# hsp-iit/roft

Measured on AMD Instinct MI355X. Metric: tracker frames/sec per object (640x480) + ADD-S vs CPU ref, higher is better.
Workload: dtype f64; 1 GPU; BASELINE config #4: 640x480, CV_32FC2 flow grid 1, 64 objects in total, 64 per GPU (sharded by object, no data-path collective; result rows all-gathered over RCCL at N > 1), masks+poses at 5 fps with 6-frame delay, flow-aided masks, re-sync and outlier rejection on, frames submitted in batches of at most 8; objects_per_gpu=64, objects_total=64, width=640, height=480, batch_frames=8, ranks=1, backend=nccl

## Files before the change

### roft_amd/csrc/batch_plan.h

```cpp
#pragma once

#include <cstdlib>

namespace roft {
namespace host {

constexpr int kPlanLanes = 2;

struct SchedKnobs {
    int handoff_mode = 1;
    int prep_mode = 1;
    int part_mode = 1;
    int feat_mask_mode = 1;
    int lanes_wait_skf = 1;
    int early_lanes = 1;
    int ctrl_ingest = 1;
    int gather_copy = 1;
    int outlier_steady_div = 2;
    bool host_prof = false;
    bool host_prof_per_batch = false;
    bool one_stream = false;
};

inline SchedKnobs knobs_from_env()
{
    SchedKnobs k;
    auto num = [](const char* name, int& v) { const char* s = getenv(name); if (s) v = atoi(s); return s != nullptr; };
    num("ROFT_HANDOFF", k.handoff_mode);
    num("ROFT_PREP_AHEAD", k.prep_mode);
    num("ROFT_MASK_PART_GATE", k.part_mode);
    num("ROFT_FEAT_ON_MASK", k.feat_mask_mode);
    if (!num("ROFT_LANES_WAIT_SKF", k.lanes_wait_skf) && getenv("ROCPROF_COUNTER_COLLECTION")) k.handoff_mode = 0;
    num("ROFT_EARLY_LANES", k.early_lanes);
    num("ROFT_CTRL_INGEST", k.ctrl_ingest);
    num("ROFT_GATHER_COPY", k.gather_copy);
    num("ROFT_OUTLIER_STEADY_DIV", k.outlier_steady_div);
    const char* hp = getenv("ROFT_HOST_PROF");
    k.host_prof = hp && hp[0] == '1';
    k.host_prof_per_batch = k.host_prof && hp[1] == '+';
    const char* one = getenv("ROFT_ONE_STREAM");
    k.one_stream = one && one[0] == '1';
    return k;
}

struct SubmitFacts {
    int T = 1;
    bool had_uploads = false;
    bool produced_flows = false;
    unsigned plain_mask_frames = 0;
    int label_sets = 0;
    int pose_masks = 0;
    int pose_resolve = 0;
    bool any_feat = false, any_feat_now = false;
    bool feat_dep_in_batch = false;
    int n_segments[kPlanLanes] = {1, 1};
    bool lin_any[kPlanLanes] = {false, false};
    int lane_objs[kPlanLanes] = {0, 0}, lane_old_first[kPlanLanes] = {0, 0};
    int relabel_wait[kPlanLanes] = {-1, -1};
};

struct PlanInputs : SubmitFacts {
    SchedKnobs knobs;
    bool multi = true;
    bool timing = false;
    int timing_level = 2;
    bool wait_value_ok = true;
    bool have_skf_started = true;
    int n_obj = 0, cus = 256;
    int batch_counter = 0, idle_mark = 0, lead = 6, completed_batches = 0;
    int outlier_bands_per_alternative = 0;
    bool conflict_free = false;
    bool up_stream_distinct = true;
    bool feat_used_two_back = false;
    bool vel_used_prev = false;
    bool done_used_relabel[kPlanLanes] = {false, false};
    int quality_frames = 0;
};

enum class Signal {
    none,
    stop,
    record,
};
// ... 17 lines not shown
    Signal ev_done = Signal::none;
};

struct BatchPlan {
    bool steady = false, handoff = false;
    bool early_lanes = false;
    bool prep = false;
    bool prep_waits_mask = false, prep_waits_feat = false;
    bool wait_up = false;
    bool try_fused = false;
    bool label_ingest = false;
    bool pose_silhouettes = false;
    bool pose_resolve = false;
    Signal ev_ctrl = Signal::none, ev_prep = Signal::none;
    bool part_gate = false;
    Signal ev_mask = Signal::none;
    FeatRun feat = FeatRun::none;
    Signal ev_feat = Signal::none;
    VelWait vel_waits = VelWait::none;
    bool feat_waits_mask = false;
    Signal ev_skf = Signal::none, ev_vel = Signal::none;
    LanePlan lane[kPlanLanes];
    int outlier_div = 1;
    bool quality = false;
    bool quality_waits_mask = false;
    bool quality_waits_lane = false;
    Signal ev_quality = Signal::none;
};

template <class AloneFn>
// ... 23 lines not shown
    }

    p.prep = batch && in.up_stream_distinct && by_mode(k.prep_mode, p.steady, !cus_to_spare);
    p.prep_waits_mask = p.prep && in.batch_counter >= 2;
    p.prep_waits_feat = p.prep_waits_mask && in.feat_used_two_back;
    p.wait_up = multi && (in.had_uploads || in.produced_flows) && !p.prep;
    p.try_fused = k.ctrl_ingest != 0 && !p.prep && in.plain_mask_frames != 0 && !in.timing;
    p.ev_ctrl = (multi && (in.T == 1 || any_early)) ? Signal::stop : Signal::none;
    p.label_ingest = in.label_sets > 0;
    p.pose_silhouettes = in.pose_masks > 0;
    p.pose_resolve = p.pose_silhouettes && in.pose_resolve > 0;
    p.ev_prep = !p.prep ? Signal::none
                : (full || (in.plain_mask_frames == 0 && !p.label_ingest && !p.pose_silhouettes)) ? Signal::record : Signal::stop;

    p.part_gate = batch && by_mode(k.part_mode, !p.steady, cus_to_spare);
    p.ev_mask = ends(multi);

    const bool feat_behind_skf = batch && !(k.feat_mask_mode == 2 || (k.feat_mask_mode == 1 && 16 * in.n_obj <= in.cus));
    p.feat = !in.any_feat ? FeatRun::none : feat_behind_skf ? FeatRun::behind_skf : FeatRun::mask_stream;
    p.ev_feat = ends(multi && p.feat == FeatRun::mask_stream);

    p.vel_waits = !multi ? VelWait::none : in.T == 1 ? VelWait::ev_ctrl : p.part_gate ? VelWait::ev_part : VelWait::ev_mask;
    p.feat_waits_mask = p.feat == FeatRun::behind_skf && p.part_gate;
    const bool lanes_wait_skf = p.feat == FeatRun::behind_skf && k.lanes_wait_skf != 0 && !own_sets;
    p.ev_skf = ends(lanes_wait_skf);
    p.ev_vel = ends(multi);

    const bool lanes_wait_feat = p.ev_feat != Signal::none && (in.T > 1 || in.any_feat_now);
    for (int l = 0; l < kPlanLanes; ++l) {
        LanePlan& lp = p.lane[l];
// ... 22 lines not shown

    p.outlier_div = (in.outlier_bands_per_alternative == 0 && p.steady && k.outlier_steady_div > 1) ? k.outlier_steady_div : 1;
    return p;
}

enum class PrepLaunch { none, mask_ingest, label_ingest, pose_silhouettes, pose_resolve };
inline PrepLaunch prep_last_launch(const BatchPlan& p, unsigned plain_mask_frames)
{
    return p.pose_resolve ? PrepLaunch::pose_resolve
           : p.pose_silhouettes ? PrepLaunch::pose_silhouettes
           : p.label_ingest ? PrepLaunch::label_ingest
           : plain_mask_frames ? PrepLaunch::mask_ingest : PrepLaunch::none;
}
inline int pose_silhouette_launches(const BatchPlan& p) { return p.pose_resolve ? 2 : p.pose_silhouettes ? 1 : 0; }

}
}
```

### roft_amd/csrc/engine_step.hip

```cpp
#include "engine_internal.h"

__global__ void ctrl_upload_kernel(const uint4* __restrict__ src, EngineArrays a, size_t n16, int reset)
{
    uint4* dst = reinterpret_cast<uint4*>(a.ctrl);
    const size_t i0 = (size_t)blockIdx.x * blockDim.x + threadIdx.x, stride = (size_t)gridDim.x * blockDim.x;
    for (size_t i = i0; i < n16; i += stride) dst[i] = src[i];
    if (reset)
        for (size_t i = i0; i < (size_t)a.T * a.n_obj; i += stride) roft::mask_reset_tables(a, i);
}


static hipEvent_t push_mark(roft_engine* e, const char* name, int which)
{
    const size_t idx = e->tmark.size();
    while (e->tev.size() <= idx) {
        hipEvent_t ev;
        (void)hipEventCreate(&ev);
        e->tev.push_back(ev);
    }
    int id = -1;
    if (name) {
        for (size_t i = 0; i < e->tnames_s.size(); ++i)
            if (e->tnames_s[i] == name) id = (int)i;
        if (id < 0) { e->tnames_s.push_back(name); id = (int)e->tnames_s.size() - 1; }
// ... 57 lines not shown
    roft_engine* e = q.e;
    const PendingBatch& pb = e->pending;
    const BatchPlan& p = q.p;
    const EngineArrays& a = q.a;
    hipStream_t s = e->stream, sp = p.prep ? e->up_stream : s;
    if (p.wait_up) TRY(q.wait(s, q.cur.ev_up));
    if (p.prep_waits_mask) {
        BatchSlot& two_back = e->slot_of(e->batch_counter - 2);
        TRY(q.wait(sp, two_back.ev_mask));
        if (p.prep_waits_feat) TRY(q.wait(sp, two_back.ev_feat));
    }
    tmark(e, nullptr, p.prep ? 4 : 0);
    static_assert(sizeof(FrameCtrl) % 16 == 0, "FrameCtrl is copied in 16-byte units");
    const size_t n16 = (sizeof(FrameCtrl) * (size_t)a.n_obj * a.T + (p.label_ingest ? pb.label_table_bytes : 0)) / 16;
    const hipEvent_t ctrl_stop = Enqueue::stop(p.ev_ctrl, q.cur.ev_ctrl);
    const PrepLaunch last_launch = prep_last_launch(p, pb.facts.plain_mask_frames);
    auto label_ingest = [&]() -> int {
        LabelIngestArgs la;
        la.sets = reinterpret_cast<const LabelSet*>(a.ctrl + (size_t)a.n_obj * a.T);
        la.members = reinterpret_cast<const LabelMember*>(la.sets + pb.label_sets.size());
        la.planes = a.planes;
        la.plane_words = a.plane_words;
        la.obj_stride = (size_t)kPlaneSlotsTotal * 2 * a.plane_words;
        la.slot0 = a.slot_new;
        la.mrec = a.mrec;
        la.n_obj = a.n_obj;
        la.n_grp = a.cam.W * a.cam.H / 64;
        launch_label_ingest(la, (int)pb.label_sets.size(), sp, last_launch == PrepLaunch::label_ingest ? Enqueue::stop(p.ev_prep, q.cur.ev_prep) : nullptr);
        ++q.launches;
        CHECK_LAUNCH("label image ingest");
// ... 30 lines not shown
            sa.zpairs = pm.zpairs.p + (size_t)(e->batch_counter & 1) * kMaxBatch * e->cfg.max_objects;
        }
        const int slot = e->batch_counter % roft_engine::kBatchRing;
        const hipEvent_t plan_stop = Enqueue::stop(p.ev_prep, q.cur.ev_prep);
        if (!p.prep) tmark(e, nullptr, 0);
        const int launched = launch_pose_silhouette(sa, n_frames, a.max_verts, 0, 1, sp, pm.ev_start[slot], plan_stop ? plan_stop : pm.ev_stop[slot]);
        if (launched != pose_silhouette_launches(p))
            return fail(ROFT_ERR_INVALID, "pose masks: the image does not fit the kernel's bit window");
        pm.last_slot = slot;
        pm.last_timed = plan_stop == nullptr;
        q.launches += launched;
        CHECK_LAUNCH(p.pose_resolve ? "pose silhouettes: clear, draw and resolve" : "pose silhouettes");
        if (!p.prep) tmark(e, "pose_silhouettes", 0);
        return ROFT_OK;
    };
    if (p.try_fused && launch_ctrl_ingest(q.cur.stage, a, n16, pb.facts.plain_mask_frames, sp, ctrl_stop)) {
        ++q.launches;
        CHECK_LAUNCH("FrameCtrl upload + mask ingest");
        if (p.label_ingest) TRY(label_ingest());
        return p.pose_silhouettes ? pose_silhouettes() : ROFT_OK;
    }
    hipExtLaunchKernelGGL(ctrl_upload_kernel, dim3((unsigned)std::min<size_t>((n16 + 255) / 256, 64)), dim3(256), 0, sp, nullptr, ctrl_stop, 0,
                          reinterpret_cast<const uint4*>(q.cur.stage), a, n16, 1);
    ++q.launches;
    CHECK_LAUNCH("FrameCtrl upload");
    int last = -1;
    for (int t = 0; t < a.T; ++t)
        if (pb.facts.plain_mask_frames & (1u << t)) last = t;
    for (int t = 0; t <= last; ++t)
        if (pb.facts.plain_mask_frames & (1u << t)) {
            launch_mask_ingest(a, t, sp, (t == last && last_launch == PrepLaunch::mask_ingest) ? Enqueue::stop(p.ev_prep, q.cur.ev_prep) : nullptr);
            ++q.launches;
        }
    CHECK_LAUNCH("mask ingest");
    if (p.label_ingest) TRY(label_ingest());
    if (p.pose_silhouettes) TRY(pose_silhouettes());
    if (p.prep) {
        TRY(q.signalled(p.ev_prep, q.cur.ev_prep, sp));
        tmark(e, "mask_prepare", 4);
        TRY(q.wait(s, q.cur.ev_prep));
    }
    return ROFT_OK;
}

static int enqueue_mask_frames(Enqueue& q)
{
    roft_engine* e = q.e;
    const BatchPlan& p = q.p;
    hipStream_t s = e->stream;
    tmark(e, nullptr, 0);
    q.launches += launch_mask_chain(q.a, e->cfg.mask_frames_between, e->cfg.flow_aided_segmentation, e->pending.new_mask_frames, s,
                                    Enqueue::stop(p.ev_mask, q.cur.ev_mask), p.part_gate ? q.cur.ev_part : nullptr);
    CHECK_LAUNCH("mask chain");
    tmark(e, "mask_chain", 0);
    TRY(q.signalled(p.ev_mask, q.cur.ev_mask, s));
    q.cur.feat_used = p.ev_feat != Signal::none;
    if (p.feat == FeatRun::mask_stream) {
        launch_features(q.a, s, Enqueue::stop(p.ev_feat, q.cur.ev_feat), e->pending.feat_frames);
        ++q.launches;
        CHECK_LAUNCH("features");
        tmark(e, "features", 0);
        TRY(q.signalled(p.ev_feat, q.cur.ev_feat, s));
    }
    return ROFT_OK;
}

static int enqueue_velocity(Enqueue& q)
{
// ... 100 lines not shown
    eq.last_slot = slot;
    return q.signalled(p.ev_quality, eq.ev_done[slot], sp);
}

static PlanInputs plan_inputs(roft_engine* e)
{
    PlanInputs in;
    static_cast<SubmitFacts&>(in) = e->pending.facts;
    in.knobs = e->knobs;
    in.multi = e->multi();
    in.timing = e->timing;
    in.timing_level = e->timing_level;
    in.wait_value_ok = e->wait_value_ok;
    in.have_skf_started = e->arr.skf_started.p != nullptr;
    in.n_obj = e->arr.a.n_obj;
    in.cus = device_cu_count();
    in.batch_counter = e->batch_counter; in.idle_mark = e->idle_mark; in.lead = e->lead; in.completed_batches = e->completed_batches;
    in.outlier_bands_per_alternative = e->cfg.outlier_bands_per_alternative;
    in.conflict_free = e->streams && e->streams->conflicts == 0;
    in.up_stream_distinct = e->up_stream != e->stream;
    if (e->quality.enabled) (void)quality_frames_of_batch(e, &in.quality_frames);
    in.feat_used_two_back = e->batch_counter >= 2 && e->slot_of(e->batch_counter - 2).feat_used;
    in.vel_used_prev = e->batch_counter >= 1 && e->slot_of(e->batch_counter - 1).vel_used;
    for (int l = 0; l < kNumLin; ++l) in.done_used_relabel[l] = in.relabel_wait[l] >= 0 && e->slot_of(in.relabel_wait[l]).done_used[1 - l];
    return in;
}

int step_batch(roft_engine* e)
{
    const PendingBatch& pb = e->pending;
// ... 112 lines not shown
```

### roft_amd/csrc/engine_submit.hip

```cpp
#include "engine_internal.h"

static void take_feat_slot(Sched& o, FrameCtrl& c)
{
    if (c.feat_write < 0) { c.feat_write = o.feat_next; o.feat_next = (o.feat_next + 1) % kFeatRing; }
    o.feat_slot = c.feat_write;
}

bool build_pose_program(const roft_config& cfg, Sched& o, const roft_frame_input& in, FrameCtrl& c)
{
    const int slot = o.frame_idx % kTwistRing;
    c.twist_slot = slot;
    int n = 0;
    bool overflow = false;
    auto add = [&](StepDesc sd) { if (n < kMaxSteps) c.steps[n++] = sd; else overflow = true; };
    auto vel_pop_front = [&]() { std::memmove(o.vel_buf, o.vel_buf + 1, sizeof(int) * (size_t)(--o.n_vel)); };

    const bool has_vel = cfg.use_velocity != 0;
    const bool is_pose = cfg.use_pose && in.pose_valid;
    int type = ROFT_MEAS_NONE;
    if (has_vel && is_pose) type = ROFT_MEAS_POSE_VELOCITY;
    else if (has_vel) type = ROFT_MEAS_VELOCITY;
    else if (is_pose) type = ROFT_MEAS_POSE;
    if (has_vel) {
        if (o.n_vel == kTwistRing) vel_pop_front();
// ... 429 lines not shown

static int schedule_mask_source(roft_engine* e, const FrameJob& j, const ImageSizes& sz, const DevInputs& d)
{
    PendingBatch& pb = e->pending;
    HostObject& ho = j.ho;
    Sched& o = ho.s;
    FrameCtrl& c = j.c;
    c.slot_prev = (o.frame_idx + kPlaneSlots - 1) % kPlaneSlots;
    c.slot_cur = o.frame_idx % kPlaneSlots;
    const EnginePoseMasks& pm = e->pose_masks;
    const bool enrolled = pm.enabled && (ho.pose_masks || (pm.all && has_mesh(e->h_params[j.id])));
    const bool from_pose = enrolled && !d.mask && !d.labels && (j.in.pose_valid || o.track_frames == 0);
    const bool has_mask = d.mask || d.labels || from_pose;
    c.has_new_mask = has_mask ? 1 : 0;
    c.new_mask = static_cast<const uint8_t*>(d.mask);
    if (has_mask) pb.new_mask_frames |= 1u << j.t;
    if (d.mask) pb.facts.plain_mask_frames |= 1u << j.t;
    if (d.labels) {
        c.label = j.lm->label;
        c.label_type = j.lm->label_type;
        int si = -1;
        for (size_t i = pb.label_sets.size(); i-- > 0 && pb.label_sets[i].t == j.t;)
            if (pb.label_sets[i].img == d.labels && pb.label_sets[i].type == j.lm->label_type) { si = (int)i; break; }
        if (si < 0) {
            LabelSet ls{};
            ls.img = d.labels; ls.type = j.lm->label_type; ls.t = j.t;
            pb.label_sets.push_back(ls);
            pb.label_members.emplace_back();
            si = pb.facts.label_sets++;
        }
        pb.label_members[si].push_back(LabelMember{j.id, j.lm->label});
    }
    if (from_pose) {
        c.label_type = kMaskFromPose;
        pb.pose_mask_frames |= 1u << j.t;
        pb.facts.pose_masks++;
    }
    if (has_mask && !o.seg_available) { o.seg_available = true; c.first_mask = 1; }
    if (!o.seg_available)
        return fail(ROFT_ERR_STATE, "no segmentation mask delivered yet: the first frame must carry one (or the object be enrolled with roft_engine_enable_pose_masks)");
    const bool valid_flow = d.flow && !o.of_first_frame;
    o.of_first_frame = false;
    if (valid_flow) {
        const int keep = std::min(o.n_hist, e->hist_cap - 1);
        std::memmove(o.hist + 1, o.hist, sizeof(FlowEntry) * (size_t)keep);
        o.hist[0] = FlowEntry{d.flow, o.frame_idx, -1, o.depth_prev};
        o.n_hist = keep + 1;
        o.flows_since_mask++;
        o.flows_buffered = std::min(o.flows_buffered + 1, kMaxFlowHist);
    }
    for (int k0 = 0; k0 < o.n_hist; ++k0) {
        FlowEntry& fe = o.hist[k0];
        if (fe.owned >= 0 || o.frame_idx - fe.frame < e->hist_cap) continue;
// ... 534 lines not shown
```

### roft_amd/csrc/k_mask.hip

```cpp
#include <algorithm>
#include <initializer_list>

#include "roft_device.h"

namespace roft {

__device__ __forceinline__ void bytes_to_bits(uint32_t w, int shift, unsigned long long& nz, unsigned long long& ob)
{
#pragma unroll
    for (int k = 0; k < 4; ++k) {
        const uint32_t v = (w >> (8 * k)) & 0xFFu;
        nz |= (unsigned long long)(v != 0u) << (shift + k);
        ob |= (unsigned long long)(v > 1u) << (shift + k);
    }
}

__device__ __forceinline__ void ingest_group(const uint4* src, int g, uint2* nz, uint2* ob, int& count, int& ones)
{
    unsigned long long bnz = 0, bob = 0;
    uint4 v[4];
#pragma unroll
    for (int q = 0; q < 4; ++q) v[q] = src[(size_t)g * 4 + q];
#pragma unroll
    for (int q = 0; q < 4; ++q) {
// ... 23 lines not shown
        atomicAdd(&r.new_count, count);
        if (ones) atomicAdd(&r.new_ones, ones);
    }
}

__global__ __launch_bounds__(256) void mask_ingest_kernel(EngineArrays a, int t)
{
    ROFT_RESIDENT(a, RK_MASK_INGEST);
    const int obj = blockIdx.y;
    const FrameCtrl& c = frame_ctrl(a, t, obj);
    if (!c.has_new_mask || c.label_type) return;
    ingest_delivered(a, c, t, obj, blockIdx.x);
}

__global__ __launch_bounds__(256) void ctrl_ingest_kernel(const uint4* __restrict__ src, EngineArrays a, size_t n16, int copy_blocks,
                                                          int chunks, unsigned frames_packed)
{
    if ((int)blockIdx.x < copy_blocks) {
        uint4* dst = reinterpret_cast<uint4*>(a.ctrl);
        const size_t stride = (size_t)copy_blocks * blockDim.x;
        for (size_t i = (size_t)blockIdx.x * blockDim.x + threadIdx.x; i < n16; i += stride) dst[i] = src[i];
        return;
    }
    ROFT_RESIDENT(a, RK_MASK_INGEST);
    const int w = (int)blockIdx.x - copy_blocks;
    const int chunk = w % chunks, rest = w / chunks, obj = rest % a.n_obj, fi = rest / a.n_obj;
    const int t = (int)((frames_packed >> (4 * fi)) & 15u);
    const FrameCtrl& c = reinterpret_cast<const FrameCtrl*>(src)[(size_t)t * a.n_obj + obj];
    if (!c.has_new_mask || c.label_type) return;
    ingest_delivered(a, c, t, obj, chunk);
}

bool launch_ctrl_ingest(const void* staging, const EngineArrays& a, size_t n16, unsigned new_mask_frames, hipStream_t s, hipEvent_t stop)
{
    unsigned packed = 0;
    int n_frames = 0;
    for (int t = 0; t < a.T && t < 16; ++t)
        if (new_mask_frames & (1u << t)) {
            if (n_frames >= 8) return false;
            packed |= (unsigned)t << (4 * n_frames++);
        }
    const int n_grp = a.cam.W * a.cam.H / 64, chunks = (n_grp + 255) / 256;
    const int copy_blocks = (int)std::min<size_t>((n16 + 255) / 256, 64);
    const unsigned grid = (unsigned)copy_blocks + (unsigned)n_frames * (unsigned)a.n_obj * (unsigned)chunks;
    hipExtLaunchKernelGGL(ctrl_ingest_kernel, dim3(grid), dim3(256), 0, s, nullptr, stop, 0, reinterpret_cast<const uint4*>(staging), a, n16,
                          copy_blocks, chunks, packed);
    return true;
}

void launch_mask_ingest(const EngineArrays& a, int t, hipStream_t s, hipEvent_t stop)
{
    const int n_grp = a.cam.W * a.cam.H / 64;
    hipExtLaunchKernelGGL(mask_ingest_kernel, dim3((n_grp + 255) / 256, a.n_obj), dim3(256), 0, s, nullptr, stop, 0, a, t);
}

__device__ __forceinline__ uint32_t eq_bits_u8(uint32_t w, uint32_t rep)
{
    const uint32_t x = w ^ rep;
    const uint32_t z = ~(((x & 0x7F7F7F7Fu) + 0x7F7F7F7Fu) | x | 0x7F7F7F7Fu);
    return ((z >> 7) * 0x01020408u) >> 24;
}
// ... 68 lines not shown
__global__ void mask_reset_kernel(EngineArrays a)
{
    mask_reset_tables(a, (size_t)blockIdx.x * blockDim.x + threadIdx.x);
}

void launch_mask_reset(const EngineArrays& a, hipStream_t s)
{
    hipLaunchKernelGGL(mask_reset_kernel, dim3(((a.T + 1) * a.n_obj + 255) / 256), dim3(256), 0, s, a);
}

constexpr int kFrameThreads = 256, kFreshThreads = 128;

struct MaskShared {
    int bbox[4];
    int n_list;
    unsigned long long w00[2];
    const void* flows[kMaxFlowHist];
};

struct ChaseGeo {
    int W, H, cols, grid;
    float grid_f, scale;
    float inv_grid, inv_scale;
    int mode;
};

__host__ __device__ inline ChaseGeo make_chase_geo(const DevCamera& cam, const DevFlowFmt& f)
{
    ChaseGeo g;
    g.W = cam.W; g.H = cam.H; g.cols = f.cols; g.grid = f.grid;
// ... 339 lines not shown
    if (flow_aided) {
        r.mode = decide_mode(c, new_slot, prev.fbuf_n, new_count, frames_between, r.src_slot, r.n_flows);
        r.fbuf_n = next_fbuf(c, prev.fbuf_n, new_count, r.mode, frames_between);
    } else {
        r.mode = 0;
        r.src_slot = c.has_new_mask ? new_slot : c.slot_prev;
        r.n_flows = 0;
        r.fbuf_n = 0;
    }
    r.src_binary = (r.src_slot >= kSlotNew) ? new_binary : prev.binary;
    r.binary = r.src_binary;
    return r;
}

#ifdef ROFT_MASK_PROFILE
#define MTICK(i) do { __syncthreads(); if (threadIdx.x == 0) atomicMax((unsigned long long*)&a.state[blockIdx.y].dbg[(i)], (unsigned long long)wall_clock64()); } while (0)
#else
#define MTICK(i) do {} while (0)
#endif

template <int FT, int THREADS>
__global__ __launch_bounds__(THREADS) __attribute__((amdgpu_waves_per_eu(4, 8)))
void mask_frame_kernel(EngineArrays a, int t, int frames_between, int flow_aided, int grp_per_wg, int margin, int win_cap)
{
#ifdef ROFT_MASK_PROFILE
    if (threadIdx.x == 0) atomicMax((unsigned long long*)&a.state[blockIdx.y].dbg[8], (unsigned long long)((1ll << 62) - wall_clock64()));
#endif
    ROFT_RESIDENT(a, THREADS == kFreshThreads ? RK_MASK_FRESH_EMPTY : RK_MASK_FRAME_EMPTY);
    extern __shared__ __attribute__((aligned(16))) unsigned char smem[];
    __shared__ MaskShared S;
    __shared__ FrameCtrl s_c;
    __shared__ MaskRec s_rec[2];
    static_assert(sizeof(MaskRec) == 32, "two 16-byte loads per record");
    uint32_t* s_win = reinterpret_cast<uint32_t*>(smem);
    uint32_t* s_list = s_win + win_cap;
    uint2* s_words = reinterpret_cast<uint2*>(s_list + THREADS);
    const int obj = blockIdx.y, q = blockIdx.x;
    const int W = a.cam.W, H = a.cam.H, wpr = a.cam.wpr, n_grp = (W * H) >> 6;
    const int tid = threadIdx.x;
    const int g0 = q * grp_per_wg, g1 = min(n_grp, g0 + grp_per_wg);
    const int r_lo = max(0, (g0 * 64) / W - margin), r_hi = min(H - 1, (g1 * 64 - 1) / W + margin);
    const int win_off = r_lo * wpr, win_words = min(win_cap, (r_hi - r_lo + 1) * wpr);
    stage_ctrl(&s_c, frame_ctrl(a, t, obj));
    if (tid >= THREADS / 2 && tid < THREADS / 2 + 4) {
        const int k = tid - THREADS / 2;
        const MaskRec* prev = (t == 0) ? a.mrec_carry + obj : a.mrec + (size_t)t * a.n_obj + obj;
        reinterpret_cast<uint4*>(s_rec)[k] = (k >= 2) ? reinterpret_cast<const uint4*>(a.mrec + (size_t)(t + 1) * a.n_obj + obj)[k & 1]
                                                      : reinterpret_cast<const uint4*>(prev)[k & 1];
    }
    const int guess_prev = a.slot_prev0 >= 0 ? (a.slot_prev0 + t) % kPlaneSlots : -1, guess_new = a.slot_new + t;
    const ROFT_GLOBAL unsigned long long* pl_prev = guess_prev >= 0 ? (const ROFT_GLOBAL unsigned long long*)(a.planes + plane_offset(a, obj, guess_prev, 1)) : nullptr;
    const ROFT_GLOBAL unsigned long long* pl_new = (const ROFT_GLOBAL unsigned long long*)(a.planes + plane_offset(a, obj, guess_new, 1));
    unsigned long long w_prev = 0ull, w_new = 0ull;
    if (g0 + tid < g1) {
        if (pl_prev) w_prev = pl_prev[g0 + tid];
        w_new = pl_new[g0 + tid];
    }
    if (tid == THREADS * 3 / 4) { S.w00[0] = pl_prev ? pl_prev[0] : 0ull; S.w00[1] = pl_new[0]; }
    for (int i = tid; i < win_words; i += THREADS) s_win[i] = 0u;
    if (tid == 0) S.n_list = 0;
    __syncthreads();
    MTICK(4);
    const FrameCtrl& c = s_c;
    const MaskRec r = decide_frame(s_rec[0], s_rec[1], a.slot_new + t, c, frames_between, flow_aided);
    if (q == 0 && tid == 0) a.mrec[(size_t)(t + 1) * a.n_obj + obj] = r;
    if (tid < kMaxFlowHist) S.flows[tid] = (tid < r.n_flows) ? c.flow[tid] : nullptr;
    MTICK(0);
    const size_t sh0 = (size_t)2 * g0, sh_n = (size_t)2 * (g1 - g0);
    plane_fill(a.planes + plane_offset(a, obj, (c.slot_cur + 1) % kPlaneSlots, 1) + sh0, 0u, sh_n);
    MTICK(5);
    const uint32_t* src = a.planes + plane_offset(a, obj, r.src_slot, 1);
    uint32_t* dst = a.planes + plane_offset(a, obj, c.slot_cur, 1);
    if (!r.src_binary) {
        if (q == 0 && tid == 0) atomicOr(&a.mask_general[obj], 1u << t);
        return;
    }
    if (r.mode == 0) {
        plane_copy(dst + sh0, src + sh0, sh_n);
        return;
    }
    const bool from_guess = r.src_slot == guess_prev || r.src_slot == guess_new;
    const unsigned long long w00 = from_guess ? S.w00[r.src_slot == guess_new ? 1 : 0] : *reinterpret_cast<const unsigned long long*>(src);
    if (r.mode == 2 && (w00 & 1ull)) {
        plane_fill(dst + sh0, ~0u, sh_n);
        return;
    }
    MTICK(6);
    const ChaseGeo geo = make_chase_geo(a.cam, a.ffmt);
// ... 24 lines not shown
        }
        __syncthreads();
        MTICK(1);
        if (S.n_list > 0) ROFT_RESIDENT_AS(a, THREADS == kFreshThreads ? RK_MASK_FRESH : RK_MASK_FRAME);
        propagate_binary<FT, THREADS / 64>(geo, plane2, s_list, S.n_list, r.n_flows, r.mode == 1, S.flows, tgt, s_words);
    }
    __syncthreads();
    MTICK(2);
    for (int i = tid; i < win_words; i += THREADS) {
        const uint32_t v = s_win[i];
        if (v) atomicOr(&dst[win_off + i], v);
    }
    MTICK(3);
}

constexpr int kMaskThreads = 256;
constexpr int kMaskWaves = kMaskThreads / 64;
constexpr int kGeneralList = 16384;
template <int FT>
__global__ __launch_bounds__(kMaskThreads) void mask_general_kernel(EngineArrays a, int final_launch)
{
    extern __shared__ __attribute__((aligned(16))) unsigned char smem[];
    __shared__ MaskShared S;
    uint32_t* s_list = reinterpret_cast<uint32_t*>(smem);
    const int obj = blockIdx.x;
    const int W = a.cam.W, H = a.cam.H, npix = W * H, n_grp = npix >> 6;
    const int tid = threadIdx.x, lane = tid & 63;
    ROFT_RESIDENT(a, RK_MASK_GENERAL);
    if (final_launch && tid < a.T) {
        MaskRec& r0 = a.mrec[(size_t)(tid + 1) * a.n_obj + obj];
        r0.new_count = 0;
        r0.new_ones = 0;
    }
    const unsigned todo = a.mask_general[obj];
    if (!todo) return;
    __syncthreads();
    if (tid == 0) a.mask_general[obj] = 0u;
    for (int t = 0; t < a.T; ++t) {
        if (!((todo >> t) & 1u)) continue;
        const MaskRec r = a.mrec[(size_t)(t + 1) * a.n_obj + obj];
        const FrameCtrl& c = frame_ctrl(a, t, obj);
        const uint32_t* snz = a.planes + plane_offset(a, obj, r.src_slot, 0);
        const uint32_t* sob = a.planes + plane_offset(a, obj, r.src_slot, 1);
        uint32_t* dnz = a.planes + plane_offset(a, obj, c.slot_cur, 0);
        uint32_t* dob = a.planes + plane_offset(a, obj, c.slot_cur, 1);
        if (r.mode == 0) {
            plane_copy(dnz, snz, a.plane_words);
            plane_copy(dob, sob, a.plane_words);
        } else {
            const bool bg_nz = (r.mode == 2) && (snz[0] & 1u), bg_ob = (r.mode == 2) && (sob[0] & 1u);
            if (tid < kMaxFlowHist) S.flows[tid] = (tid < r.n_flows) ? c.flow[tid] : nullptr;
            if (tid == 0) { S.n_list = 0; S.bbox[0] = INT32_MAX; S.bbox[1] = INT32_MAX; S.bbox[2] = -1; S.bbox[3] = -1; }
            __syncthreads();
            const uint2* plane2 = reinterpret_cast<const uint2*>(snz);
            int32_t* map = a.map + (size_t)obj * npix;
            for (int c0 = 0; c0 < n_grp; c0 += kGeneralList) {
                const int c1 = min(n_grp, c0 + kGeneralList);
                for (int g0 = c0; g0 < c1; g0 += kMaskThreads) {
// ... 22 lines not shown
                        obb = (sob[m >> 5] >> (m & 31)) & 1u;
                    }
                }
                const unsigned long long b1 = __ballot(nzb), b2 = __ballot(obb);
                if (lane == 0) {
                    reinterpret_cast<uint2*>(dnz)[g] = make_uint2((uint32_t)b1, (uint32_t)(b1 >> 32));
                    reinterpret_cast<uint2*>(dob)[g] = make_uint2((uint32_t)b2, (uint32_t)(b2 >> 32));
                }
            }
        }
        __syncthreads();
    }
}

int launch_mask_chain(const EngineArrays& a, int frames_between, int flow_aided, unsigned new_mask_frames, hipStream_t s, hipEvent_t stop,
                      hipEvent_t stop_early)
{
    const int n_grp = a.cam.W * a.cam.H / 64;
    constexpr int kBandRows = 20, kBandRowsFresh = 6;
    auto per_for = [&](bool fresh) {
        if (a.mask_wgs > 0) return (n_grp + a.mask_wgs - 1) / a.mask_wgs;
        const int per = std::max(1, (fresh ? kBandRowsFresh : kBandRows) * a.cam.W / 64);
        return std::min(per, n_grp);
    };
    const size_t lds_cap = 160 * 1024 - 4096;
    auto frame_kernel = [](bool s16, int threads) {
        if (threads == kFrameThreads) return s16 ? mask_frame_kernel<ROFT_FLOW_S16C2, kFrameThreads> : mask_frame_kernel<ROFT_FLOW_F32C2, kFrameThreads>;
        return s16 ? mask_frame_kernel<ROFT_FLOW_S16C2, kFreshThreads> : mask_frame_kernel<ROFT_FLOW_F32C2, kFreshThreads>;
    };
    auto general_kernel = [](bool s16) { return s16 ? mask_general_kernel<ROFT_FLOW_S16C2> : mask_general_kernel<ROFT_FLOW_F32C2>; };
    for (int threads : {kFrameThreads, kFreshThreads})
        for (bool f16 : {true, false}) (void)set_max_dynamic_lds(reinterpret_cast<const void*>(frame_kernel(f16, threads)), (int)lds_cap);
    int launches = 0;
    const bool s16 = a.ffmt.type == ROFT_FLOW_S16C2;
    auto launch_general = [&](hipEvent_t ev, int final_launch) {
        const size_t lds_gen = ((size_t)std::min(n_grp, kGeneralList) * 4 + 15) & ~(size_t)15;
        for (bool f16 : {true, false}) (void)set_max_dynamic_lds(reinterpret_cast<const void*>(general_kernel(f16)), kGeneralList * 4 + 16);
        hipExtLaunchKernelGGL(general_kernel(s16), dim3(a.n_obj), dim3(kMaskThreads), (uint32_t)lds_gen, s, nullptr, ev, 0, a, final_launch);
    };
    for (int t = 0; t < a.T; ++t) {
        const bool fresh = (new_mask_frames >> t) & 1u;
        const int per = per_for(fresh);
        constexpr int kMargin = 16, kMarginFresh = 48;
        const int margin = fresh ? kMarginFresh : kMargin;
        const int threads = fresh ? kFreshThreads : kFrameThreads;
        const size_t fixed = (size_t)threads * 12;
        size_t win_cap = ((size_t)std::min(a.cam.H, (per * 64 + a.cam.W - 1) / a.cam.W + 1 + 2 * margin) * a.cam.wpr + 1) & ~(size_t)1;
        win_cap = std::min(win_cap, ((lds_cap - fixed) / 4) & ~(size_t)1);
        const size_t lds = win_cap * 4 + fixed;
        const dim3 grid((n_grp + per - 1) / per, a.n_obj);
        hipLaunchKernelGGL(frame_kernel(s16, threads), grid, dim3(threads), (uint32_t)lds, s, a, t, frames_between, flow_aided, per, margin, (int)win_cap);
        ++launches;
        if (stop_early && t == a.T - 2) { launch_general(stop_early, 0); ++launches; }
    }
    launch_general(stop, 1);
    return launches + 1;
}

__global__ __launch_bounds__(256) void plane_to_mask_kernel(const uint32_t* nz, const uint32_t* ob, int npix,
                                                            uint8_t* mask)
{
    const int p = blockIdx.x * blockDim.x + threadIdx.x;
    if (p >= npix) return;
    const bool o = (ob[p >> 5] >> (p & 31)) & 1u;
    const bool n = nz ? ((nz[p >> 5] >> (p & 31)) & 1u) : false;
    mask[p] = o ? 255 : (n ? 1 : 0);
}

// ... 7 lines not shown
```

### roft_amd/csrc/roft_device.h

```cpp
#pragma once

#include <hip/hip_runtime.h>
#include <hip/hip_ext.h>
#include <stdint.h>

#include "../../include/roft_engine.h"

namespace roft {

constexpr int kWave = 64;
constexpr int kNumLin = 2;
constexpr int kNumBelief = 9;
constexpr int kMaxBatch = ROFT_MAX_BATCH_FRAMES;
constexpr int kTwistRing = 64;
constexpr int kMaxFlowHist = ROFT_MAX_FLOW_CHASE;
constexpr int kMaxOutlierParts = 8;
constexpr int kMaxSteps = 10;
constexpr int kPlaneSlots = 64;
constexpr int kFeatRing = 12;

enum BeliefSlot { B_LIN0 = 0, B_LIN1 = 1, B_PRED = 2 , B_ALT0 = 4 , B_ALT1 = 5 ,
                  B_SPARE = 8, B_CORR = B_LIN0  };
__host__ __device__ inline int b_alt(int lane, int k) { return B_ALT0 + 2 * lane + k; }

// ... 260 lines not shown

__device__ inline int next_fbuf(const FrameCtrl& c, int fbuf_n, int new_count, int mode, int frames_between)
{
    if (c.has_new_mask && !c.first_mask && new_count == 0 && frames_between <= 0) fbuf_n = 0;
    int n = fbuf_n + (c.flow_valid ? 1 : 0);
    if (n > kMaxFlowHist) n = kMaxFlowHist;
    return (mode == 2) ? 0 : n;
}

__host__ __device__ inline size_t plane_offset(const EngineArrays& a, int obj, int slot, int which)
{
    return (((size_t)obj * kPlaneSlotsTotal + slot) * 2 + which) * a.plane_words;
}

void launch_mask_ingest(const EngineArrays& a, int t, hipStream_t s, hipEvent_t stop = nullptr);
bool launch_ctrl_ingest(const void* staging, const EngineArrays& a, size_t n16, unsigned new_mask_frames, hipStream_t s, hipEvent_t stop = nullptr);
struct alignas(16) LabelSet {
    const void* img;
    int type;
    int t;
    int first, n;
};
struct LabelMember { int obj, label; };
struct LabelIngestArgs {
    const LabelSet* sets;
    const LabelMember* members;
    uint32_t* planes;
    size_t obj_stride, plane_words;
    int slot0;
    MaskRec* mrec;
    int n_obj, n_grp;
// ... 31 lines not shown
    unsigned long long* gstats;
    int* gremoved;
};
int launch_pose_silhouette(SilhouetteArgs sa, int n_frames, int max_verts, int bands, int vertex_cache, hipStream_t s,
                            hipEvent_t start = nullptr, hipEvent_t stop = nullptr);
void launch_mask_reset(const EngineArrays& a, hipStream_t s);
__device__ inline void mask_reset_tables(const EngineArrays& a, size_t i)
{
    if (i < (size_t)a.T * a.n_obj) {
        MaskRec& r = a.mrec[(size_t)a.n_obj + i];
        r.new_count = 0;
        r.new_ones = 0;
    }
}
int launch_mask_chain(const EngineArrays& a, int frames_between, int flow_aided, unsigned new_mask_frames, hipStream_t s, hipEvent_t stop = nullptr,
                      hipEvent_t stop_early = nullptr);
void launch_planes_to_mask(const uint32_t* nz, const uint32_t* ob, int npix, uint8_t* mask, hipStream_t s);
void launch_flow_measure(const EngineArrays& a, double depth_max, int radius, hipStream_t s,
                         hipEvent_t start = nullptr, hipEvent_t stop = nullptr);
void launch_skf_chain(const EngineArrays& a, int reweight, hipStream_t s, hipEvent_t stop = nullptr);
void launch_skf_arrays(const double* x_pred, const double* P_pred, int N, const double* y, const double* H,
                       const double* Rdiag, int reweight, double* norms, double* x_out, double* P_out, int* status,
                       hipStream_t s);
void launch_skf_records(const double* x_pred, const double* P_pred, int N, const FlowRec* recs, DevCamera cam, double dt,
                        const double* Rdiag, int reweight, double* norms, double* x_out, double* P_out, int* status,
                        hipStream_t s);
void launch_kf_predict(const double* x, const double* P, const double* qdiag, double* xo, double* Po, hipStream_t s);
void launch_ukf_chain(const EngineArrays& a, roft_ut_params ut, bool first_segment, int lin, hipStream_t s, hipEvent_t stop = nullptr);
void launch_features(const EngineArrays& a, hipStream_t s, hipEvent_t stop = nullptr, unsigned feat_frames = 0);
struct OutlierLaunchOpts {
    int parts = 0;
// ... 30 lines not shown
```

Measured before the change: 1.791 million object-frames/s.

## Pair the mask-delivery frame with frame 0 in one mask chain launch

```diff
diff --git a/roft_amd/csrc/batch_plan.h b/roft_amd/csrc/batch_plan.h
--- a/roft_amd/csrc/batch_plan.h
+++ b/roft_amd/csrc/batch_plan.h
@@ -16,6 +16,7 @@
     int early_lanes = 1;
     int ctrl_ingest = 1;
     int gather_copy = 1;
+    int mask_pair = 1;
     int outlier_steady_div = 2;
     bool host_prof = false;
     bool host_prof_per_batch = false;
@@ -34,6 +35,7 @@
     num("ROFT_EARLY_LANES", k.early_lanes);
     num("ROFT_CTRL_INGEST", k.ctrl_ingest);
     num("ROFT_GATHER_COPY", k.gather_copy);
+    num("ROFT_MASK_PAIR", k.mask_pair);
     num("ROFT_OUTLIER_STEADY_DIV", k.outlier_steady_div);
     const char* hp = getenv("ROFT_HOST_PROF");
     k.host_prof = hp && hp[0] == '1';
@@ -48,6 +50,8 @@
     bool had_uploads = false;
     bool produced_flows = false;
     unsigned plain_mask_frames = 0;
+    unsigned delivering_frames = 0;
+    bool first_mask_delivery = false;
     int label_sets = 0;
     int pose_masks = 0;
     int pose_resolve = 0;
@@ -67,6 +71,8 @@
     bool wait_value_ok = true;
     bool have_skf_started = true;
     int n_obj = 0, cus = 256;
+    bool flow_aided = true;
+    bool mask_force_mode = false;
     int batch_counter = 0, idle_mark = 0, lead = 6, completed_batches = 0;
     int outlier_bands_per_alternative = 0;
     bool conflict_free = false;
@@ -114,6 +120,7 @@
     bool pose_resolve = false;
     Signal ev_ctrl = Signal::none, ev_prep = Signal::none;
     bool part_gate = false;
+    int mask_pair_frame = -1;
     Signal ev_mask = Signal::none;
     FeatRun feat = FeatRun::none;
     Signal ev_feat = Signal::none;
@@ -167,6 +174,13 @@
                 : (full || (in.plain_mask_frames == 0 && !p.label_ingest && !p.pose_silhouettes)) ? Signal::record : Signal::stop;
 
     p.part_gate = batch && by_mode(k.part_mode, !p.steady, cus_to_spare);
+    {
+        const unsigned d = in.delivering_frames & ((in.T >= 32) ? ~0u : ((1u << in.T) - 1u));
+        const bool one = d != 0u && (d & (d - 1u)) == 0u;
+        if (batch && in.flow_aided && k.mask_pair != 0 && one && !(d & 1u) && !in.first_mask_delivery && !in.mask_force_mode)
+            for (int t = 1; t < in.T; ++t)
+                if (d >> t & 1u) p.mask_pair_frame = t;
+    }
     p.ev_mask = ends(multi);
 
     const bool feat_behind_skf = batch && !(k.feat_mask_mode == 2 || (k.feat_mask_mode == 1 && 16 * in.n_obj <= in.cus));
@@ -219,5 +233,8 @@
 }
 inline int pose_silhouette_launches(const BatchPlan& p) { return p.pose_resolve ? 2 : p.pose_silhouettes ? 1 : 0; }
 
-}
-}
+inline int mask_chain_launches(const BatchPlan& p, int T) { return T - (p.mask_pair_frame >= 1 ? 1 : 0) + 1 + (p.part_gate ? 1 : 0); }
+inline int mask_part_frame(const BatchPlan& p, int T) { return (T - 2 == p.mask_pair_frame) ? T - 3 : T - 2; }
+
+}
+}
diff --git a/roft_amd/csrc/engine_step.hip b/roft_amd/csrc/engine_step.hip
--- a/roft_amd/csrc/engine_step.hip
+++ b/roft_amd/csrc/engine_step.hip
@@ -1,12 +1,13 @@
 #include "engine_internal.h"
 
-__global__ void ctrl_upload_kernel(const uint4* __restrict__ src, EngineArrays a, size_t n16, int reset)
+__global__ void ctrl_upload_kernel(const uint4* __restrict__ src, EngineArrays a, size_t n16, int reset, int zero_slot)
 {
     uint4* dst = reinterpret_cast<uint4*>(a.ctrl);
     const size_t i0 = (size_t)blockIdx.x * blockDim.x + threadIdx.x, stride = (size_t)gridDim.x * blockDim.x;
     for (size_t i = i0; i < n16; i += stride) dst[i] = src[i];
     if (reset)
         for (size_t i = i0; i < (size_t)a.T * a.n_obj; i += stride) roft::mask_reset_tables(a, i);
+    if (zero_slot >= 0) roft::mask_zero_slot(a, zero_slot, i0, stride);
 }
 
 
@@ -95,6 +96,7 @@
     static_assert(sizeof(FrameCtrl) % 16 == 0, "FrameCtrl is copied in 16-byte units");
     const size_t n16 = (sizeof(FrameCtrl) * (size_t)a.n_obj * a.T + (p.label_ingest ? pb.label_table_bytes : 0)) / 16;
     const hipEvent_t ctrl_stop = Enqueue::stop(p.ev_ctrl, q.cur.ev_ctrl);
+    const int zero_slot = p.mask_pair_frame >= 1 ? (e->frame_counter + p.mask_pair_frame) % kPlaneSlots : -1;
     const PrepLaunch last_launch = prep_last_launch(p, pb.facts.plain_mask_frames);
     auto label_ingest = [&]() -> int {
         LabelIngestArgs la;
@@ -155,14 +157,14 @@
         if (!p.prep) tmark(e, "pose_silhouettes", 0);
         return ROFT_OK;
     };
-    if (p.try_fused && launch_ctrl_ingest(q.cur.stage, a, n16, pb.facts.plain_mask_frames, sp, ctrl_stop)) {
+    if (p.try_fused && launch_ctrl_ingest(q.cur.stage, a, n16, pb.facts.plain_mask_frames, sp, ctrl_stop, zero_slot)) {
         ++q.launches;
         CHECK_LAUNCH("FrameCtrl upload + mask ingest");
         if (p.label_ingest) TRY(label_ingest());
         return p.pose_silhouettes ? pose_silhouettes() : ROFT_OK;
     }
     hipExtLaunchKernelGGL(ctrl_upload_kernel, dim3((unsigned)std::min<size_t>((n16 + 255) / 256, 64)), dim3(256), 0, sp, nullptr, ctrl_stop, 0,
-                          reinterpret_cast<const uint4*>(q.cur.stage), a, n16, 1);
+                          reinterpret_cast<const uint4*>(q.cur.stage), a, n16, 1, zero_slot);
     ++q.launches;
     CHECK_LAUNCH("FrameCtrl upload");
     int last = -1;
@@ -190,9 +192,11 @@
     const BatchPlan& p = q.p;
     hipStream_t s = e->stream;
     tmark(e, nullptr, 0);
-    q.launches += launch_mask_chain(q.a, e->cfg.mask_frames_between, e->cfg.flow_aided_segmentation, e->pending.new_mask_frames, s,
-                                    Enqueue::stop(p.ev_mask, q.cur.ev_mask), p.part_gate ? q.cur.ev_part : nullptr);
+    const int chain = launch_mask_chain(q.a, e->cfg.mask_frames_between, e->cfg.flow_aided_segmentation, e->pending.new_mask_frames, s,
+                                        Enqueue::stop(p.ev_mask, q.cur.ev_mask), p.part_gate ? q.cur.ev_part : nullptr, p.mask_pair_frame);
+    q.launches += chain;
     CHECK_LAUNCH("mask chain");
+    if (chain != mask_chain_launches(p, q.a.T)) return fail(ROFT_ERR_STATE, "mask chain: the launches enqueued are not the plan's");
     tmark(e, "mask_chain", 0);
     TRY(q.signalled(p.ev_mask, q.cur.ev_mask, s));
     q.cur.feat_used = p.ev_feat != Signal::none;
@@ -323,6 +327,7 @@
     in.wait_value_ok = e->wait_value_ok;
     in.have_skf_started = e->arr.skf_started.p != nullptr;
     in.n_obj = e->arr.a.n_obj;
+    in.flow_aided = e->cfg.flow_aided_segmentation != 0;
     in.cus = device_cu_count();
     in.batch_counter = e->batch_counter; in.idle_mark = e->idle_mark; in.lead = e->lead; in.completed_batches = e->completed_batches;
     in.outlier_bands_per_alternative = e->cfg.outlier_bands_per_alternative;
diff --git a/roft_amd/csrc/engine_submit.hip b/roft_amd/csrc/engine_submit.hip
--- a/roft_amd/csrc/engine_submit.hip
+++ b/roft_amd/csrc/engine_submit.hip
@@ -467,7 +467,7 @@
     const bool has_mask = d.mask || d.labels || from_pose;
     c.has_new_mask = has_mask ? 1 : 0;
     c.new_mask = static_cast<const uint8_t*>(d.mask);
-    if (has_mask) pb.new_mask_frames |= 1u << j.t;
+    if (has_mask) { pb.new_mask_frames |= 1u << j.t; pb.facts.delivering_frames |= 1u << j.t; }
     if (d.mask) pb.facts.plain_mask_frames |= 1u << j.t;
     if (d.labels) {
         c.label = j.lm->label;
@@ -489,7 +489,7 @@
         pb.pose_mask_frames |= 1u << j.t;
         pb.facts.pose_masks++;
     }
-    if (has_mask && !o.seg_available) { o.seg_available = true; c.first_mask = 1; }
+    if (has_mask && !o.seg_available) { o.seg_available = true; c.first_mask = 1; pb.facts.first_mask_delivery = true; }
     if (!o.seg_available)
         return fail(ROFT_ERR_STATE, "no segmentation mask delivered yet: the first frame must carry one (or the object be enrolled with roft_engine_enable_pose_masks)");
     const bool valid_flow = d.flow && !o.of_first_frame;
diff --git a/roft_amd/csrc/k_mask.hip b/roft_amd/csrc/k_mask.hip
--- a/roft_amd/csrc/k_mask.hip
+++ b/roft_amd/csrc/k_mask.hip
@@ -61,12 +61,13 @@
 }
 
 __global__ __launch_bounds__(256) void ctrl_ingest_kernel(const uint4* __restrict__ src, EngineArrays a, size_t n16, int copy_blocks,
-                                                          int chunks, unsigned frames_packed)
+                                                          int chunks, unsigned frames_packed, int zero_slot)
 {
     if ((int)blockIdx.x < copy_blocks) {
         uint4* dst = reinterpret_cast<uint4*>(a.ctrl);
         const size_t stride = (size_t)copy_blocks * blockDim.x;
         for (size_t i = (size_t)blockIdx.x * blockDim.x + threadIdx.x; i < n16; i += stride) dst[i] = src[i];
+        if (zero_slot >= 0) mask_zero_slot(a, zero_slot, (size_t)blockIdx.x * blockDim.x + threadIdx.x, stride);
         return;
     }
     ROFT_RESIDENT(a, RK_MASK_INGEST);
@@ -78,7 +79,7 @@
     ingest_delivered(a, c, t, obj, chunk);
 }
 
-bool launch_ctrl_ingest(const void* staging, const EngineArrays& a, size_t n16, unsigned new_mask_frames, hipStream_t s, hipEvent_t stop)
+bool launch_ctrl_ingest(const void* staging, const EngineArrays& a, size_t n16, unsigned new_mask_frames, hipStream_t s, hipEvent_t stop, int zero_slot)
 {
     unsigned packed = 0;
     int n_frames = 0;
@@ -91,7 +92,7 @@
     const int copy_blocks = (int)std::min<size_t>((n16 + 255) / 256, 64);
     const unsigned grid = (unsigned)copy_blocks + (unsigned)n_frames * (unsigned)a.n_obj * (unsigned)chunks;
     hipExtLaunchKernelGGL(ctrl_ingest_kernel, dim3(grid), dim3(256), 0, s, nullptr, stop, 0, reinterpret_cast<const uint4*>(staging), a, n16,
-                          copy_blocks, chunks, packed);
+                          copy_blocks, chunks, packed, zero_slot);
     return true;
 }
 
@@ -190,6 +191,7 @@
 struct MaskShared {
     int bbox[4];
     int n_list;
+    int flows_before;
     unsigned long long w00[2];
     const void* flows[kMaxFlowHist];
 };
@@ -559,17 +561,17 @@
 }
 
 #ifdef ROFT_MASK_PROFILE
-#define MTICK(i) do { __syncthreads(); if (threadIdx.x == 0) atomicMax((unsigned long long*)&a.state[blockIdx.y].dbg[(i)], (unsigned long long)wall_clock64()); } while (0)
+#define MTICK(i) do { __syncthreads(); if (threadIdx.x == 0) atomicMax((unsigned long long*)&a.state[obj].dbg[(i)], (unsigned long long)wall_clock64()); } while (0)
 #else
 #define MTICK(i) do {} while (0)
 #endif
 
 template <int FT, int THREADS>
-__global__ __launch_bounds__(THREADS) __attribute__((amdgpu_waves_per_eu(4, 8)))
-void mask_frame_kernel(EngineArrays a, int t, int frames_between, int flow_aided, int grp_per_wg, int margin, int win_cap)
+__device__ __forceinline__ void mask_frame_band(const EngineArrays& a, int t, int obj, int q, int frames_between, int flow_aided, int grp_per_wg,
+                                                int margin, int win_cap, bool keep_next, bool deliver)
 {
 #ifdef ROFT_MASK_PROFILE
-    if (threadIdx.x == 0) atomicMax((unsigned long long*)&a.state[blockIdx.y].dbg[8], (unsigned long long)((1ll << 62) - wall_clock64()));
+    if (threadIdx.x == 0) atomicMax((unsigned long long*)&a.state[obj].dbg[8], (unsigned long long)((1ll << 62) - wall_clock64()));
 #endif
     ROFT_RESIDENT(a, THREADS == kFreshThreads ? RK_MASK_FRESH_EMPTY : RK_MASK_FRAME_EMPTY);
     extern __shared__ __attribute__((aligned(16))) unsigned char smem[];
@@ -580,7 +582,6 @@
     uint32_t* s_win = reinterpret_cast<uint32_t*>(smem);
     uint32_t* s_list = s_win + win_cap;
     uint2* s_words = reinterpret_cast<uint2*>(s_list + THREADS);
-    const int obj = blockIdx.y, q = blockIdx.x;
     const int W = a.cam.W, H = a.cam.H, wpr = a.cam.wpr, n_grp = (W * H) >> 6;
     const int tid = threadIdx.x;
     const int g0 = q * grp_per_wg, g1 = min(n_grp, g0 + grp_per_wg);
@@ -589,11 +590,15 @@
     stage_ctrl(&s_c, frame_ctrl(a, t, obj));
     if (tid >= THREADS / 2 && tid < THREADS / 2 + 4) {
         const int k = tid - THREADS / 2;
-        const MaskRec* prev = (t == 0) ? a.mrec_carry + obj : a.mrec + (size_t)t * a.n_obj + obj;
+        const MaskRec* prev = (t == 0 || deliver) ? a.mrec_carry + obj : a.mrec + (size_t)t * a.n_obj + obj;
         reinterpret_cast<uint4*>(s_rec)[k] = (k >= 2) ? reinterpret_cast<const uint4*>(a.mrec + (size_t)(t + 1) * a.n_obj + obj)[k & 1]
                                                       : reinterpret_cast<const uint4*>(prev)[k & 1];
     }
-    const int guess_prev = a.slot_prev0 >= 0 ? (a.slot_prev0 + t) % kPlaneSlots : -1, guess_new = a.slot_new + t;
+    if (deliver && tid < 64) {
+        const int n = __popcll(__ballot(tid < t && frame_ctrl(a, tid, obj).flow_valid != 0));
+        if (tid == 0) S.flows_before = n;
+    }
+    const int guess_prev = (a.slot_prev0 >= 0 && !deliver) ? (a.slot_prev0 + t) % kPlaneSlots : -1, guess_new = a.slot_new + t;
     const ROFT_GLOBAL unsigned long long* pl_prev = guess_prev >= 0 ? (const ROFT_GLOBAL unsigned long long*)(a.planes + plane_offset(a, obj, guess_prev, 1)) : nullptr;
     const ROFT_GLOBAL unsigned long long* pl_new = (const ROFT_GLOBAL unsigned long long*)(a.planes + plane_offset(a, obj, guess_new, 1));
     unsigned long long w_prev = 0ull, w_new = 0ull;
@@ -607,16 +612,20 @@
     __syncthreads();
     MTICK(4);
     const FrameCtrl& c = s_c;
-    const MaskRec r = decide_frame(s_rec[0], s_rec[1], a.slot_new + t, c, frames_between, flow_aided);
+    MaskRec before = s_rec[0];
+    if (deliver) before.fbuf_n = min(before.fbuf_n + S.flows_before, kMaxFlowHist);
+    MaskRec r = decide_frame(before, s_rec[1], a.slot_new + t, c, frames_between, flow_aided);
+    const bool hand_over = deliver && !(r.src_slot == guess_new && r.src_binary);
+    if (hand_over) r.binary = 0;
     if (q == 0 && tid == 0) a.mrec[(size_t)(t + 1) * a.n_obj + obj] = r;
     if (tid < kMaxFlowHist) S.flows[tid] = (tid < r.n_flows) ? c.flow[tid] : nullptr;
     MTICK(0);
     const size_t sh0 = (size_t)2 * g0, sh_n = (size_t)2 * (g1 - g0);
-    plane_fill(a.planes + plane_offset(a, obj, (c.slot_cur + 1) % kPlaneSlots, 1) + sh0, 0u, sh_n);
+    if (!keep_next) plane_fill(a.planes + plane_offset(a, obj, (c.slot_cur + 1) % kPlaneSlots, 1) + sh0, 0u, sh_n);
     MTICK(5);
     const uint32_t* src = a.planes + plane_offset(a, obj, r.src_slot, 1);
     uint32_t* dst = a.planes + plane_offset(a, obj, c.slot_cur, 1);
-    if (!r.src_binary) {
+    if (!r.src_binary || hand_over) {
         if (q == 0 && tid == 0) atomicOr(&a.mask_general[obj], 1u << t);
         return;
     }
@@ -671,6 +680,30 @@
     MTICK(3);
 }
 
+template <int FT, int THREADS>
+__global__ __launch_bounds__(THREADS) __attribute__((amdgpu_waves_per_eu(4, 8)))
+void mask_frame_kernel(EngineArrays a, int t, int frames_between, int flow_aided, int grp_per_wg, int margin, int win_cap, int keep_next)
+{
+    mask_frame_band<FT, THREADS>(a, t, blockIdx.y, blockIdx.x, frames_between, flow_aided, grp_per_wg, margin, win_cap, keep_next != 0, false);
+}
+
+struct MaskPairArgs {
+    int q_ord, q_del;
+    int t_d;
+    int grp_per_wg, margin;
+};
+template <int FT>
+__global__ __launch_bounds__(kFrameThreads) __attribute__((amdgpu_waves_per_eu(4, 8)))
+void mask_pair_kernel(EngineArrays a, int frames_between, int grp_per_wg, int margin, int win_cap, MaskPairArgs pa)
+{
+    const int n_del = pa.q_del * a.n_obj;
+    const bool deliver = (int)blockIdx.x < n_del;
+    const int i = deliver ? (int)blockIdx.x : (int)blockIdx.x - n_del, per_obj = deliver ? pa.q_del : pa.q_ord;
+    const int obj = i / per_obj;
+    mask_frame_band<FT, kFrameThreads>(a, deliver ? pa.t_d : 0, obj, i - obj * per_obj, frames_between, 1, deliver ? pa.grp_per_wg : grp_per_wg,
+                                       deliver ? pa.margin : margin, win_cap, !deliver && pa.t_d == 1, deliver);
+}
+
 constexpr int kMaskThreads = 256;
 constexpr int kMaskWaves = kMaskThreads / 64;
 constexpr int kGeneralList = 16384;
@@ -697,8 +730,8 @@
         if (!((todo >> t) & 1u)) continue;
         const MaskRec r = a.mrec[(size_t)(t + 1) * a.n_obj + obj];
         const FrameCtrl& c = frame_ctrl(a, t, obj);
-        const uint32_t* snz = a.planes + plane_offset(a, obj, r.src_slot, 0);
         const uint32_t* sob = a.planes + plane_offset(a, obj, r.src_slot, 1);
+        const uint32_t* snz = r.src_binary ? sob : a.planes + plane_offset(a, obj, r.src_slot, 0);
         uint32_t* dnz = a.planes + plane_offset(a, obj, c.slot_cur, 0);
         uint32_t* dob = a.planes + plane_offset(a, obj, c.slot_cur, 1);
         if (r.mode == 0) {
@@ -751,7 +784,7 @@
 }
 
 int launch_mask_chain(const EngineArrays& a, int frames_between, int flow_aided, unsigned new_mask_frames, hipStream_t s, hipEvent_t stop,
-                      hipEvent_t stop_early)
+                      hipEvent_t stop_early, int pair_frame)
 {
     const int n_grp = a.cam.W * a.cam.H / 64;
     constexpr int kBandRows = 20, kBandRowsFresh = 6;
@@ -775,20 +808,45 @@
         for (bool f16 : {true, false}) (void)set_max_dynamic_lds(reinterpret_cast<const void*>(general_kernel(f16)), kGeneralList * 4 + 16);
         hipExtLaunchKernelGGL(general_kernel(s16), dim3(a.n_obj), dim3(kMaskThreads), (uint32_t)lds_gen, s, nullptr, ev, 0, a, final_launch);
     };
+    constexpr int kMargin = 16, kMarginFresh = 48;
+    auto window_cap = [&](int per, int margin) {
+        return ((size_t)std::min(a.cam.H, (per * 64 + a.cam.W - 1) / a.cam.W + 1 + 2 * margin) * a.cam.wpr + 1) & ~(size_t)1;
+    };
+    const int t_part = (a.T - 2 == pair_frame) ? a.T - 3 : a.T - 2;
     for (int t = 0; t < a.T; ++t) {
+        if (t == pair_frame) continue;
+        if (t == 0 && pair_frame > 0) {
+            const int per = per_for(false);
+            MaskPairArgs pa;
+            pa.q_ord = (n_grp + per - 1) / per;
+            pa.t_d = pair_frame;
+            pa.grp_per_wg = a.mask_wgs > 0 ? per_for(true) : std::min(2 * per_for(true), n_grp);
+            pa.q_del = (n_grp + pa.grp_per_wg - 1) / pa.grp_per_wg;
+            pa.margin = kMarginFresh;
+            const size_t fixed = (size_t)kFrameThreads * 12;
+            size_t win_cap = std::max(window_cap(per, kMargin), window_cap(pa.grp_per_wg, pa.margin));
+            win_cap = std::min(win_cap, ((lds_cap - fixed) / 4) & ~(size_t)1);
+            const size_t lds = win_cap * 4 + fixed;
+            auto pair_kernel = s16 ? mask_pair_kernel<ROFT_FLOW_S16C2> : mask_pair_kernel<ROFT_FLOW_F32C2>;
+            (void)set_max_dynamic_lds(reinterpret_cast<const void*>(pair_kernel), (int)lds_cap);
+            const dim3 grid((unsigned)(pa.q_ord + pa.q_del) * (unsigned)a.n_obj);
+            hipLaunchKernelGGL(pair_kernel, grid, dim3(kFrameThreads), (uint32_t)lds, s, a, frames_between, per, kMargin, (int)win_cap, pa);
+            ++launches;
+            if (stop_early && t == t_part) { launch_general(stop_early, 0); ++launches; }
+            continue;
+        }
         const bool fresh = (new_mask_frames >> t) & 1u;
         const int per = per_for(fresh);
-        constexpr int kMargin = 16, kMarginFresh = 48;
         const int margin = fresh ? kMarginFresh : kMargin;
         const int threads = fresh ? kFreshThreads : kFrameThreads;
         const size_t fixed = (size_t)threads * 12;
-        size_t win_cap = ((size_t)std::min(a.cam.H, (per * 64 + a.cam.W - 1) / a.cam.W + 1 + 2 * margin) * a.cam.wpr + 1) & ~(size_t)1;
-        win_cap = std::min(win_cap, ((lds_cap - fixed) / 4) & ~(size_t)1);
+        const size_t win_cap = std::min(window_cap(per, margin), ((lds_cap - fixed) / 4) & ~(size_t)1);
         const size_t lds = win_cap * 4 + fixed;
         const dim3 grid((n_grp + per - 1) / per, a.n_obj);
-        hipLaunchKernelGGL(frame_kernel(s16, threads), grid, dim3(threads), (uint32_t)lds, s, a, t, frames_between, flow_aided, per, margin, (int)win_cap);
+        hipLaunchKernelGGL(frame_kernel(s16, threads), grid, dim3(threads), (uint32_t)lds, s, a, t, frames_between, flow_aided, per, margin, (int)win_cap,
+                           (t + 1 == pair_frame) ? 1 : 0);
         ++launches;
-        if (stop_early && t == a.T - 2) { launch_general(stop_early, 0); ++launches; }
+        if (stop_early && t == t_part) { launch_general(stop_early, 0); ++launches; }
     }
     launch_general(stop, 1);
     return launches + 1;
diff --git a/roft_amd/csrc/roft_device.h b/roft_amd/csrc/roft_device.h
--- a/roft_amd/csrc/roft_device.h
+++ b/roft_amd/csrc/roft_device.h
@@ -298,7 +298,8 @@
 }
 
 void launch_mask_ingest(const EngineArrays& a, int t, hipStream_t s, hipEvent_t stop = nullptr);
-bool launch_ctrl_ingest(const void* staging, const EngineArrays& a, size_t n16, unsigned new_mask_frames, hipStream_t s, hipEvent_t stop = nullptr);
+bool launch_ctrl_ingest(const void* staging, const EngineArrays& a, size_t n16, unsigned new_mask_frames, hipStream_t s, hipEvent_t stop = nullptr,
+                        int zero_slot = -1);
 struct alignas(16) LabelSet {
     const void* img;
     int type;
@@ -360,7 +361,16 @@
     }
 }
 int launch_mask_chain(const EngineArrays& a, int frames_between, int flow_aided, unsigned new_mask_frames, hipStream_t s, hipEvent_t stop = nullptr,
-                      hipEvent_t stop_early = nullptr);
+                      hipEvent_t stop_early = nullptr,
+                      int pair_frame = -1);
+__device__ inline void mask_zero_slot(const EngineArrays& a, int slot, size_t i0, size_t stride)
+{
+    const size_t per = a.plane_words / 2;
+    for (size_t i = i0; i < per * (size_t)a.n_obj; i += stride) {
+        const size_t obj = i / per;
+        reinterpret_cast<uint2*>(a.planes + plane_offset(a, (int)obj, slot, 1))[i - obj * per] = make_uint2(0u, 0u);
+    }
+}
 void launch_planes_to_mask(const uint32_t* nz, const uint32_t* ob, int npix, uint8_t* mask, hipStream_t s);
 void launch_flow_measure(const EngineArrays& a, double depth_max, int radius, hipStream_t s,
                          hipEvent_t start = nullptr, hipEvent_t stop = nullptr);
```

Result: slower. 1.766 million object-frames/s (-1.4%).
